# nebarnix/Project-Desert-Tortoise

Measured on AMD Instinct MI355X. Metric: IQ Msamples/s end-to-end (WAV→minorframes), 1-GPU + %HBM roofline, higher is better.
Workload: dtype f32

## Files before the change

project-desert-tortoise_amd/csrc/pdt_api.hip:

```cpp
#include "pdt_rt.h"
#include "pdt_analytic.h"
#include "pdt_ddc.h"
#include "pdt_survey.h"
#include "pdt_bursts.h"

#include <pthread.h>
#include <sched.h>
#include <sys/mman.h>
#include <sys/stat.h>
#include <sys/syscall.h>

namespace pdtrt {
PDT_CHAIN_INSTANCES(extern, float)
PDT_CHAIN_INSTANCES(extern, double)
std::atomic<long long> g_alloc_ns{0};
hipError_t analytic_launch(hipStream_t st, int fmt, const void *x, long long lo, long long hi, unsigned long long n_out, unsigned long long g0,
                           uint32_t step, const float *tab_dev, void *out);
size_t survey_part_floats(uint64_t nseg, int nfft);
hipError_t survey_launch(hipStream_t st, int fmt, const void *x, uint64_t nseg, int nfft, const float *win, const float *tw, float *part, float *out);
int survey_plan(const pdt_survey_cfg *cfg, double mode_range_hz, double channel_rate, uint64_t nframes, int cap, pdt::SurveyPlan *p);
int survey_carriers(const float *P, const pdt::SurveyPlan &p, double in_rate, pdt_carrier *found);
hipError_t waterfall_launch(hipStream_t st, int fmt, const void *x, uint64_t nrows, int rows_per, int nfft, const float *win, const float *tw, float *rows);
hipError_t row_peaks_launch(hipStream_t st, const float *rows, uint64_t nrows, int nfft, float level, int gb, void *peaks, int *counts);
int bursts_plan(const pdt_bursts_cfg *cfg, double mode_range_hz, double channel_rate, double in_rate, uint64_t nframes, int cap, pdt::BurstPlan *p);
pdt::SurveyPlan bursts_survey_plan(const pdt::BurstPlan &p, const pdt_bursts_cfg *cfg, uint64_t nframes);
int bursts_link(const void *peaks, const int *counts, bool compact, const pdt::BurstPlan &p, double floor, double in_rate, pdt_burst *found, int cap);
hipError_t ddc_launch(hipStream_t st, int fmt, const void *x, long long lo, long long hi, unsigned long long n_out, unsigned long long g0,
                      int decim, const float *taps_dev, const float *tab_dev, const uint32_t *steps, void *const *outs, int k);
}

static std::atomic<int> g_open_contexts{0};
static std::mutex g_link_mu[64];

static std::mutex g_dev_mu;
static std::map<std::string, std::string> g_dev;
void Tuning::load()
{
    std::lock_guard<std::mutex> lock(g_dev_mu);
    if (g_dev.empty()) return;
    auto get = [&](const char *n) -> const char * { auto it = g_dev.find(n); return it == g_dev.end() ? nullptr : it->second.c_str(); };
    if (const char *e = get("PDT_PLL_WARM_SCALE")) pll_warm_scale = atof(e);
    if (const char *e = get("PDT_HEAD_TAUS")) head_taus = atof(e);
    if (const char *e = get("PDT_BAND_PAD")) band_pad = atof(e);
    if (const char *e = get("PDT_PLL_WARM_S")) pll_warm_s = atof(e);
    if (const char *e = get("PDT_AGC_WARM_S")) agc_warm_s = atof(e);
    if (const char *e = get("PDT_AGC_K")) agc_k = atof(e);
    if (const char *e = get("PDT_AGC_TPB")) agc_tpb = std::max(1, atoi(e));
    if (const char *e = get("PDT_PLL_BLOCK")) pll_block = atoi(e);
    if (const char *e = get("PDT_HBM_LIMIT_MB")) hbm_limit_mb = std::max(1ll, atoll(e));
    if (const char *e = get("PDT_BURST_SLAB_ROWS")) burst_slab_rows = std::max(1ll, atoll(e));
    if (const char *e = get("PDT_WINDOW_PIECE")) window_piece = std::max(1ll, atoll(e));
    if (const char *e = get("PDT_SCOUT_SYMS")) scout_syms = std::max(16, atoi(e));
    if (const char *e = get("PDT_FIR_WG_PER_CU")) fir_wg_per_cu = std::min(4096, std::max(1, atoi(e)));
    if (const char *e = get("PDT_INGEST_THREADS")) ingest_threads = std::min(128, std::max(1, atoi(e)));
    if (const char *e = get("PDT_INGEST_SPAN_MB")) ingest_span_mb = std::min(256, std::max(1, atoi(e)));
    if (const char *e = get("PDT_INGEST_STREAMS")) ingest_streams = std::min(4, std::max(1, atoi(e)));
    if (const char *e = get("PDT_INGEST_DIRECT")) ingest_direct = atoi(e) ? 1 : 0;
    if (const char *e = get("PDT_INGEST_NUMA")) ingest_numa = atoi(e) ? 1 : 0;
    if (const char *e = get("PDT_FIX_PASSES")) fix_passes = atoi(e);
    if (const char *e = get("PDT_GSEG")) gseg = std::min(64, std::max(2, atoi(e)));
    if (const char *e = get("PDT_GSPAN")) gspan = std::min(256, std::max(1, atoi(e)));
    if (const char *e = get("PDT_GSPAN_CAP")) gspan_cap = std::max(64, atoi(e));
    fir_generic = get("PDT_FIR_GENERIC") != nullptr;
    mix_unfused = get("PDT_MIX_UNFUSED") != nullptr;
    quality_inline = get("PDT_QUALITY_INLINE") != nullptr;
    gardner_nostride = get("PDT_GARDNER_NOSTRIDE") != nullptr;
    gemit_groups = get("PDT_GEMIT_GROUPS") != nullptr;
    agc_unfused = get("PDT_AGC_UNFUSED") != nullptr;
    manch_3pass = get("PDT_MANCH_3PASS") != nullptr;
    sync_serial = get("PDT_SYNC_SERIAL") != nullptr;
    agc_lanes = get("PDT_AGC_LANES") != nullptr;
    no_excl = get("PDT_NO_EXCL") != nullptr;
    gardner_onebuf = get("PDT_GARDNER_ONEBUF") != nullptr;
    gardner_noring = get("PDT_GARDNER_NORING") != nullptr;
    ema_noguess = get("PDT_EMA_NOGUESS") != nullptr;
    gardner_sequential = get("PDT_GARDNER_SEQUENTIAL") != nullptr;
    seg_sequential = get("PDT_SEG_SEQUENTIAL") != nullptr;
    overlap = get("PDT_NO_OVERLAP") == nullptr;
    if (const char *e = get("PDT_OVERLAP_SPLIT")) {
        int k = 0;
        for (const char *q = e; *q && k < 8; k++) {
            char *end = nullptr;
            overlap_split[k] = strtod(q, &end);
            if (end == q) break;
            q = (*end == ',') ? end + 1 : end;
        }
    }
    chain_one_range = get("PDT_CHAIN_ONE_RANGE") != nullptr;
    debug_overlap = get("PDT_DEBUG_OVERLAP") != nullptr;
    if (const char *e = get("PDT_OVERLAP_SEGMENTS")) overlap_segments = std::min(64, std::max(1, atoi(e)));
    if (const char *e = get("PDT_OVERLAP_MIN_MB")) overlap_min_mb = std::min(1 << 20, std::max(1, atoi(e)));
    debug_sync = get("PDT_DEBUG_SYNC") != nullptr;
    pll_noshort = get("PDT_PLL_NOSHORT") != nullptr;
    pll_nockpt = get("PDT_PLL_NOCKPT") != nullptr;
    pll_noconsensus = get("PDT_PLL_NOCONSENSUS") != nullptr;
    pll_notail = get("PDT_PLL_NOTAIL") != nullptr;
    seg_plain = get("PDT_SEG_PLAIN") != nullptr;
    sync_block = get("PDT_SYNC_BLOCK") != nullptr;
}

namespace pdtrt {

int execute_plans(pdt_ctx *const *ctxs, int M)
{
    pdt_ctx *L0 = ctxs[0];
    HIP_TRY(hipSetDevice(L0->cfg.device));
    const Plan &P0 = L0->plan;
    for (int m = 1; m < M; m++)
        if (!P0.same_shape(ctxs[m]->plan)) return PDT_ERR_STATE;
    const size_t per = P0.packs.size();
    const size_t total = per * (size_t)M;
    int rc;
    if ((rc = L0->packs_dev.ensure(total + 64))) return rc;
    if (total + 64 > L0->packs_pin_cap) {
        if (L0->packs_pin) (void)hipHostFree(L0->packs_pin);
        L0->packs_pin = nullptr;
        L0->packs_pin_cap = 0;
        const size_t want = 2 * total + 4096;
        if (timed_host_malloc((void **)&L0->packs_pin, want) != hipSuccess) { (void)hipGetLastError(); return PDT_ERR_NOMEM; }
        L0->packs_pin_cap = want;
    }
    unsigned char *pin = (unsigned char *)L0->packs_pin;
    for (const PlanOp &o : P0.ops) {
        if (o.op != OP_LAUNCH) continue;
        for (int m = 0; m < M; m++)
            memcpy(pin + (size_t)M * o.pack_off + (size_t)m * o.pack_size, ctxs[m]->plan.packs.data() + o.pack_off, o.pack_size);
    }
    hipStream_t st[2] = { L0->stream, L0->stream2 };
    if (total) HIP_TRY(hipMemcpyAsync(L0->packs_dev.p, pin, total, hipMemcpyHostToDevice, st[0]));
    Launcher T(L0);
    const unsigned char *dev = (const unsigned char *)L0->packs_dev.p;
    for (size_t i = 0; i < P0.ops.size(); i++) {
        const PlanOp &o = P0.ops[i];
        switch (o.op) {
        case OP_LAUNCH: {
            dim3 g = o.grid;
            for (int m = 1; m < M; m++) {
                const dim3 gm = ctxs[m]->plan.ops[i].grid;
                g.x = std::max(g.x, gm.x);
                g.y = std::max(g.y, gm.y);
            }
            g.z = (unsigned)M;
            o.go(g, o.block, o.shmem, st[o.side], dev + (size_t)M * o.pack_off);
            if (L0->tune.debug_sync) {
                const hipError_t e = hipStreamSynchronize(st[o.side]);
                fprintf(stderr, "libpdt: [%zu] %s grid (%u,%u,%u) block %u lds %zu: %s\n", i, o.name, g.x, g.y, g.z, o.block.x, o.shmem,
                        hipGetErrorString(e));
            }
            break;
        }
        case OP_MEMSET:
            for (int m = 0; m < M; m++) {
                const PlanOp &om = ctxs[m]->plan.ops[i];
                if (om.bytes) HIP_TRY(hipMemsetAsync(om.dst, om.value, om.bytes, st[om.side]));
            }
            T.gap();
            break;
        case OP_D2H:
        case OP_H2D:
            for (int m = 0; m < M; m++) {
                const PlanOp &om = ctxs[m]->plan.ops[i];
                if (om.bytes)
                    HIP_TRY(hipMemcpyAsync(om.dst, om.src, om.bytes, o.op == OP_D2H ? hipMemcpyDeviceToHost : hipMemcpyHostToDevice, st[0]));
            }
            T.gap();
            break;
        case OP_FORK:
            HIP_TRY(hipEventRecord(L0->ev_fork, st[0]));
            HIP_TRY(hipStreamWaitEvent(st[1], L0->ev_fork, 0));
            break;
        case OP_JOIN_RECORD: HIP_TRY(hipEventRecord(L0->ev_join, st[1])); break;
// ... 2294 lines not shown
```

project-desert-tortoise_amd/csrc/pdt_chain.inc:

```
#include "pdt_rt.h"

namespace pdtrt {
PDT_WIDE_INSTANCES(extern, float)
PDT_WIDE_INSTANCES(extern, double)

template <typename T> int finish_capture(pdt_ctx *ctx, uint64_t n, const FinishArgs &FA)
{
    const bool argos = FA.argos, need_lock = FA.need_lock, fuse_mix = FA.fuse_mix;
    const long long N = FA.N, n_out = FA.n_out, chunk = FA.chunk, chunk_out = FA.chunk_out, first = FA.first, first_out = FA.first_out,
                    sym_cap = FA.sym_cap;
    const int interp = FA.interp, ntaps = FA.ntaps;
    const uint32_t hit_cap = FA.hit_cap, frame_cap = FA.frame_cap;
    const SyncParams &SP = FA.SP;
    const T Fs = (T)ctx->cfg.sample_rate;
    StreamCarry *seg = ctx->sc.active ? &ctx->sc : nullptr;
    FrameRec *d_frames = (FrameRec *)ctx->frames.p;
    (void)first_out;
    if (!ctx->pending || ctx->pend_n != n) return PDT_ERR_STATE;
    ctx->pending = false;
    pdt_ctx *lead = ctx->leader ? ctx->leader : ctx;
    if (seg && seg->in_place && !ctx->tune.sync_block) {
        for (;;) {
            const hipError_t e = hipEventQuery(lead->ev1);
            if (e == hipSuccess) break;
// ... 1112 lines not shown
        if constexpr (std::is_same<T, float>::value) {
            std::vector<unsigned> cand;
            std::vector<int> mfirst((size_t)GD.n_q + 1);
            cand.reserve((size_t)GD.n_q * 2);
            for (int m = 0; m < GD.n_q; m++) {
                mfirst[(size_t)m] = (int)cand.size();
                const float q = GD.q_min + (float)m * GD.u;
                const float fr = q - floorf(q);
                if (fr <= 0.61f) cand.push_back((unsigned)(2 * m));
                if (fr >= 0.39f) cand.push_back((unsigned)(2 * m + 1));
            }
            mfirst[(size_t)GD.n_q] = (int)cand.size();
            GD.n_cand = (int)cand.size();
            const long long key = chunk_out * 1000003ll + (long long)llround((double)GP.step * 4096.0);
            if ((rc = ctx->gcand.ensure(cand.size() * sizeof(unsigned)))) return rc;
            if ((rc = ctx->gmfirst.ensure(mfirst.size() * sizeof(int)))) return rc;
            if (ctx->gcand_key != key) {
                HIP_TRY(hipMemcpyAsync(ctx->gcand.p, cand.data(), cand.size() * sizeof(unsigned), hipMemcpyHostToDevice, st));
                HIP_TRY(hipMemcpyAsync(ctx->gmfirst.p, mfirst.data(), mfirst.size() * sizeof(int), hipMemcpyHostToDevice, st));
                HIP_TRY(hipStreamSynchronize(st));
                ctx->gcand_key = key;
            }
            const long long n_tab = (n_chunks - 1) / GD.span;
            const long long n_groups = n_tab + 1;
            SamplerCarry<float> tab_carry;
            tab_carry.a = (float)carry_in.a; tab_carry.b = (float)carry_in.b; tab_carry.c = (float)carry_in.c;
            tab_carry.c_first = carry_in.c_first; tab_carry.count0 = carry_in.count0;
            SamplerCarry<float> chain_carry = tab_carry;
            chain_carry.c_first = tab_carry.c_first / GD.span;
            const long long g_first = chain_carry.c_first;
            if ((rc = ctx->gtable.ensure((size_t)n_tab * (size_t)(2 * GD.n_q) * sizeof(unsigned)))) return rc;
            if ((rc = ctx->gentries.ensure((size_t)n_chunks * sizeof(GardnerEntry<float>)))) return rc;
            if ((rc = ctx->gbands.ensure((size_t)n_tab * sizeof(GardnerBand)))) return rc;
            L.begin("gardner_table");
            if ((rc = ctx->gclist.ensure((size_t)n_tab * PDT_GTAB_LIST * sizeof(unsigned)))) return rc;
            const int scout_syms = ctx->tune.scout_syms > 0 ? ctx->tune.scout_syms : 455;
            const int scout_tail = (int)std::min<long long>(PDT_GTAB_TAIL, std::max<long long>(256, (long long)((double)scout_syms * (double)GP.step) + 16));
            PDT_LAUNCH(64, k_gardner_scout, dim3((unsigned)n_tab), dim3(64), 0, st, (const float *)d_agc, GP, GD, n_tab,
                               (const int *)ctx->gmfirst.p, (const unsigned *)ctx->gcand.p, (unsigned *)ctx->gtable.p,
                               (GardnerBand *)ctx->gbands.p, (unsigned *)ctx->gclist.p, d_sc->gstats, scout_tail);
            {
                {
                    const unsigned parts = (unsigned)((GD.n_cand + PDT_GTM_SLOTS - 1) / PDT_GTM_SLOTS);
                    PDT_LAUNCH(PDT_GTM_THREADS, (k_gardner_table_merge<PDT_GTAB_WIN>), dim3((unsigned)n_tab, parts), dim3(PDT_GTM_THREADS), 0, st,
                                       (const float *)d_agc, GP, GD, n_tab, (const unsigned *)ctx->gcand.p,
                                       (const GardnerBand *)ctx->gbands.p, (const unsigned *)ctx->gclist.p,
                                       (unsigned *)ctx->gtable.p, d_sc->gstats);
                }
                if (GD.span > 1) {
                    const unsigned cap_keys = ctx->tune.gspan_cap ? (unsigned)ctx->tune.gspan_cap
                                                                  : (unsigned)std::min<long long>(std::max<long long>(n_tab * 128, 1ll << 20), 1ll << 28);
                    const size_t cap_items = (size_t)cap_keys / PDT_GSUB_KEYS + (size_t)n_tab + 1;
                    if ((rc = ctx->gspan_keys.ensure((size_t)cap_keys * sizeof(unsigned)))) return rc;
                    if ((rc = ctx->gspan_tails.ensure((size_t)cap_keys * sizeof(unsigned)))) return rc;
                    if ((rc = ctx->gspan_recs.ensure((size_t)cap_keys * (size_t)(GD.span - 1) * sizeof(GardnerSpanRec)))) return rc;
                    if ((rc = ctx->gspan_rows.ensure((size_t)n_tab * sizeof(GardnerSpanRow)))) return rc;
                    if ((rc = ctx->gspan_items.ensure(cap_items * sizeof(GardnerSpanItem)))) return rc;
                    if ((rc = ctx->gspan_ctl.ensure(sizeof(GardnerSpanCtl)))) return rc;
                    PL.memset_async(ctx->gspan_ctl.p, 0, sizeof(GardnerSpanCtl));
                    PDT_LAUNCH(256, k_gardner_span_keys, dim3((unsigned)n_tab), dim3(256), 0, st, GD, n_tab, (const unsigned *)ctx->gcand.p,
                                       (GardnerBand *)ctx->gbands.p, (const unsigned *)ctx->gclist.p, (const unsigned *)ctx->gtable.p,
                                       (unsigned *)ctx->gspan_keys.p, cap_keys, (GardnerSpanRow *)ctx->gspan_rows.p,
                                       (GardnerSpanItem *)ctx->gspan_items.p, (GardnerSpanCtl *)ctx->gspan_ctl.p);
                    const unsigned walkers = (unsigned)std::min<long long>(n_tab / PDT_GSUB + 64, 256ll * 16);
                    PDT_LAUNCH(64, (k_gardner_span_walk<PDT_GSUB_WIN>), dim3(walkers), dim3(64), 0, st, (const float *)d_agc, GP, GD,
                                       (const unsigned *)ctx->gspan_keys.p, (const GardnerSpanItem *)ctx->gspan_items.p,
                                       (GardnerSpanCtl *)ctx->gspan_ctl.p, (unsigned *)ctx->gspan_tails.p, (GardnerSpanRec *)ctx->gspan_recs.p);
                    PDT_LAUNCH(128, k_gardner_span_join, dim3((unsigned)n_tab), dim3(128), 0, st, GD, n_tab, (const unsigned *)ctx->gcand.p,
                                       (const GardnerBand *)ctx->gbands.p, (const unsigned *)ctx->gclist.p, (unsigned *)ctx->gtable.p,
                                       (const unsigned *)ctx->gspan_keys.p, (const unsigned *)ctx->gspan_tails.p,
                                       (const GardnerSpanRow *)ctx->gspan_rows.p, d_sc->gstats);
                }
            }
            L.end();
            int G = (n_groups < 8000) ? 32 : 64;
            if (ctx->tune.gseg) G = ctx->tune.gseg;
            const long long n_seg = (n_groups + G - 1) / G;
            if ((rc = ctx->gsegmap.ensure((size_t)n_seg * (size_t)(2 * GD.n_q) * sizeof(GardnerSegCell)))) return rc;
            if ((rc = ctx->gsegstart.ensure((size_t)n_seg * sizeof(GardnerSegStart)))) return rc;
            L.begin("gardner_chain");
            PL.memset_async(ctx->gsegstart.p, 0, (size_t)n_seg * sizeof(GardnerSegStart));
            PDT_LAUNCH(1024, k_gardner_segmap, dim3((unsigned)n_seg), dim3(1024), 0, st, (const unsigned *)ctx->gtable.p, GD, n_groups,
                               G, (GardnerSegCell *)ctx->gsegmap.p, (const GardnerBand *)ctx->gbands.p);
            const int n_ranges = (!seg && n_groups >= 8192 && GD.span == 1 && !ctx->tune.chain_one_range) ? 4 : 1;
            if ((rc = ctx->gchain.ensure(sizeof(GardnerChainState)))) return rc;
            const bool side = n_ranges > 1;
            hipStream_t st_emit = side ? ctx->stream2 : st;
            L.end();
            long long c_lo = 0;
            for (int r = 0; r < n_ranges; r++) {
                const long long c_hi = (r == n_ranges - 1) ? n_groups : (n_groups * (r + 1) / n_ranges) / G * G;
                L.begin("gardner_chain");
                PDT_LAUNCH(256, k_gardner_chain, dim3(1), dim3(256), 0, st,
                                   (const float *)d_agc, GP, GD, n_groups,
                                   (const unsigned *)ctx->gtable.p, (const GardnerSegCell *)ctx->gsegmap.p, G,
                                   (GardnerSegStart *)ctx->gsegstart.p, (GardnerEntry<float> *)ctx->gentries.p, d_sc->gstats,
                                   (const GardnerBand *)ctx->gbands.p, n_tab, chain_carry, (seg && seg->have_sampler) ? 1 : 0, c_hi,
                                   (GardnerChainState *)ctx->gchain.p, r == 0 ? 1 : 0,
                                   (const unsigned *)(GD.span > 1 ? ctx->gspan_keys.p : nullptr), (const unsigned *)(GD.span > 1 ? ctx->gspan_tails.p : nullptr),
                                   (const GardnerSpanRow *)(GD.span > 1 ? ctx->gspan_rows.p : nullptr));
                L.end();
                if (side) PL.simple(OP_FORK);
                const long long s_lo = c_lo / G, s_hi = (c_hi + G - 1) / G;
                L.begin("gardner", st_emit);
                if (s_hi > s_lo)
                    PDT_LAUNCH(64, k_gardner_segfill, dim3((unsigned)(s_hi - s_lo)), dim3(64), 0, st_emit, (const float *)d_agc, GP, GD, n_groups,
                                       (const unsigned *)ctx->gtable.p, G, (const GardnerSegStart *)ctx->gsegstart.p,
                                       (GardnerEntry<float> *)ctx->gentries.p, s_lo);
                const unsigned char *d_flags = nullptr;
                if (GD.span > 1 && 8 * (long long)GP.step + 256 < PDT_GEMIT_SUB_WIN && !ctx->tune.gemit_groups &&
                    (double)PDT_GEMIT_SUB_WIN / ((double)GP.step - 0.2) + 2.0 < (double)PDT_GSUB_OUT) {
                    if ((rc = ctx->gcentries.ensure((size_t)n_chunks * sizeof(GardnerEntry<float>)))) return rc;
                    if ((rc = ctx->gflags.ensure((size_t)n_groups + 64))) return rc;
                    PL.memset_async(ctx->gflags.p, 1, (size_t)n_groups, PL.side_of(st_emit));
                    PDT_LAUNCH(64, (k_gardner_emit_first<PDT_GEMIT_SUB_WIN>), dim3((unsigned)((n_tab - g_first + 3) / 4)), dim3(64), 0, st_emit, (const float *)d_agc, GP, GD,
                                       n_tab, (const GardnerEntry<float> *)ctx->gentries.p, (const unsigned *)ctx->gspan_keys.p,
                                       (const GardnerSpanRow *)ctx->gspan_rows.p, (const GardnerSpanRec *)ctx->gspan_recs.p,
                                       (GardnerEntry<float> *)ctx->gcentries.p, (unsigned char *)ctx->gflags.p, (float *)d_sym, d_symidx, sym_cap, g_first);
                    PDT_LAUNCH(64, (k_gardner_emit_rest<PDT_GEMIT_SUB_WIN>), dim3((unsigned)(((n_tab - g_first) * (GD.span - 1) + 3) / 4)), dim3(64), 0, st_emit,
                                       (const float *)d_agc, GP, GD, n_tab, (const GardnerEntry<float> *)ctx->gcentries.p,
                                       (const unsigned char *)ctx->gflags.p, (float *)d_sym, d_symidx, sym_cap, g_first);
                    d_flags = (const unsigned char *)ctx->gflags.p;
                }
                if (c_hi > c_lo)
                    PDT_LAUNCH(256, (k_gardner<float, PDT_GEMIT_LEN, PDT_GEMIT_OUT>), dim3((unsigned)(c_hi - c_lo)), dim3(PDT_GARDNER_THREADS), 0, st_emit,
                                       (const float *)d_agc, (const float *)d_lock, GP, (float *)d_sym, d_symidx, &d_sc->nsym, sym_cap,
                                       (const GardnerEntry<float> *)ctx->gentries.p, tab_carry, (SamplerCarry<float> *)d_carry_out, c_lo, GD.span, d_flags);
                L.end();
                c_lo = c_hi;
            }
            if (side) {
                PL.simple(OP_JOIN_RECORD);
                PL.simple(OP_JOIN_WAIT);
            }
        }
        return PDT_OK;
    }

    int rec_sampler()
    {
        int rc = PDT_OK;
        (void)rc;
        if (use_table) {
            if ((rc = rec_sampler_table())) return rc;
        } else if (use_mm) {
            MmParams<T> MP;
            const T rangeT = (T)(ctx->cfg.mm_step_range != 0 ? ctx->cfg.mm_step_range : 3.0);
            MP.kp = (T)(ctx->cfg.mm_kp != 0 ? ctx->cfg.mm_kp : 0.15);
            MP.step0 = (T)(int)fsi / baud;
            MP.step_max = (T)(int)fsi / (baud - rangeT);
            MP.step_min = (T)(int)fsi / (baud + rangeT);
            MP.n_total = n_out;
            MP.chunk_out = chunk_out;
            L.begin("gardner");
            if (seg && !seg->have_sampler) carry_in.b = MP.step0;
            PDT_LAUNCH(PDT_GARDNER_THREADS, (k_mm<T, 8192, 1024>), dim3(1), dim3(PDT_GARDNER_THREADS), 0, st, (const T *)d_agc, MP, d_sym, d_symidx,
                               &d_sc->nsym, sym_cap, carry_in, seg ? 1 : 0, d_carry_out);
            L.end();
        } else {
            L.begin("gardner");
            constexpr int SMALL_LEN = 32768 / (int)sizeof(T), SMALL_OUT = 1024;
            const long long small_need = chunk_out + 2 * (long long)GP.step + 24;
            const double small_syms = (double)chunk_out / ((double)GP.step - 0.25) + 4.0;
            constexpr int RING_LEN = 20480 / (int)sizeof(T), RING_NB = 6, RING_OUT = 256;
            if (small_need <= RING_LEN && small_syms < RING_OUT && chunk_out >= 4 * (long long)GP.step + 8 && n_chunks >= 8 && !seg &&
                !ctx->tune.gardner_onebuf && !ctx->tune.gardner_noring) {
                const size_t need_bytes = ((size_t)n_chunks + 64 + 15) & ~(size_t)15;
                if ((rc = ctx->gneed.ensure(need_bytes + (size_t)n_chunks * sizeof(CalmEntry<T>)))) return rc;
                CalmEntry<T> *d_calm = (CalmEntry<T> *)((char *)ctx->gneed.p + need_bytes);
                PDT_LAUNCH(256, k_chunk_need<T>, dim3((unsigned)n_chunks), dim3(256), 0, st, (const T *)d_agc, n_out, chunk_out, n_chunks,
                                   (unsigned char *)ctx->gneed.p);
                T gran_scale = 0;
                if (!ctx->tune.gardner_nostride) {
                    const double top = (double)chunk_out + 2.0 * (double)GP.step + 2.0;
                    const int E = ilogb(top) + 1, p = sizeof(T) == 8 ? 53 : 24;
                    const T sc = (T)ldexp(1.0, p - E);
                    const T gstep = GP.step * sc;
                    if (E < p && gstep == (T)rint((double)gstep) && (double)gstep < ldexp(1.0, p - 1)) gran_scale = sc;
                }
                PDT_LAUNCH(64 * (RING_NB + 1), (k_gardner_ring<T, RING_LEN, RING_NB, RING_OUT>), dim3(1), dim3(64 * (RING_NB + 1)), 0, st,
                                   (const T *)d_agc, (const T *)d_lock, GP, (const unsigned char *)ctx->gneed.p, d_sym, d_symidx, &d_sc->nsym,
                                   sym_cap, d_calm, gran_scale);
                PDT_LAUNCH(256, k_calm_emit<T>, dim3((unsigned)((n_chunks + 255) / 256)), dim3(256), 0, st, (const unsigned char *)ctx->gneed.p,
                                   (const CalmEntry<T> *)d_calm, GP, d_sym, d_symidx, sym_cap);
            } else if (small_need <= SMALL_LEN && small_syms < SMALL_OUT && !ctx->tune.gardner_onebuf && !seg)
                PDT_LAUNCH(256, (k_gardner_small<T, SMALL_LEN, SMALL_OUT>), dim3(1), dim3(256), 0, st, (const T *)d_agc, (const T *)d_lock, GP,
                                   d_sym, d_symidx, &d_sc->nsym, sym_cap);
            else
                PDT_LAUNCH(256, (k_gardner<T, GardnerLds<T>::LEN, GardnerLds<T>::OUT>), dim3(1), dim3(256), 0, st, d_agc, d_lock, GP, d_sym, d_symidx,
                                   &d_sc->nsym, sym_cap, (const GardnerEntry<T> *)nullptr, carry_in, d_carry_out, 0ll, 1, (const unsigned char *)nullptr);
            L.end();
        }

        return PDT_OK;
    }

    int rec_bits()
    {
        int rc = PDT_OK;
        (void)rc;
        L.begin("manchester");
        if (ctx->tune.manch_3pass) {
            PDT_LAUNCH(PDT_TILE_THREADS, k_manch_tile<T>, dim3((unsigned)n_tiles), dim3(PDT_TILE_THREADS), 0, st, d_sym, &d_sc->nsym, manch_thr,
                               d_tiles, sym_pad);
// ... 580 lines not shown
```

project-desert-tortoise_amd/csrc/pdt_kernels_back.h:

```cpp
#pragma once
#include "pdt_device_math.h"

namespace pdt {

template <typename T> struct alignas(16) Vec16 {
    static constexpr int N = 16 / sizeof(T);
    T v[N];
};

template <typename T> struct GardnerParams {
    T step, kp, lim;
    long long n_total;
    long long chunk_out;
    int argos_heap;
    unsigned long long argos_field_bits;
    int argos_even;
};

template <typename T>
__device__ __forceinline__ T gardner_beyond(const T *__restrict__ in, const T *__restrict__ lock, const GardnerParams<T> &P,
                                            long long c, long long n_cur, long long idx)
{
    const long long C = P.chunk_out;
    if (idx < C)
// ... 1431 lines not shown
            emit(cur, (unsigned)rn);
            const float err = __builtin_amdgcn_fmed3f(kp * (cur - L.prev) * mid, -lim, lim);
            L.ns = L.ns - err;
            L.q_last = L.ns;
            L.half = L.ns + hs;
            L.ns = L.ns + step;
            L.prev = cur;
            L.i_last = (unsigned)rn;
            L.count++;
        }
        flush();
        if (last_window) break;
        enter_hi = stop + step + 1.2f;
        wbase = wend - margin - back;
    }
}


template <int WIN>
__device__ __forceinline__ void k_gardner_span_walk(const float *__restrict__ in, GardnerParams<float> P, GardnerDomain D,
                                                    const unsigned *__restrict__ keys, const GardnerSpanItem *__restrict__ items,
                                                    GardnerSpanCtl *__restrict__ ctl, unsigned *__restrict__ tails,
                                                    GardnerSpanRec *__restrict__ recs )
{
    __shared__ __attribute__((aligned(16))) float win[PDT_GSUB * WIN];
    __shared__ float s_ref[3];
    __shared__ unsigned s_next;
    const int lane = threadIdx.x;
    const int mysub = lane / PDT_GSUB_KEYS, sublane = lane % PDT_GSUB_KEYS;
    const float nT = (float)P.chunk_out;
    const unsigned n_items = ctl->items;
    for (;;) {
        __syncthreads();
        if (lane == 0) s_next = atomicAdd(&ctl->cursor, (unsigned)PDT_GSUB);
        __syncthreads();
        const unsigned q0 = s_next;
        if (q0 >= n_items) break;
        long long c_sub[PDT_GSUB];
        GardnerSpanItem mine = items[q0];
#pragma unroll
        for (int u = 0; u < PDT_GSUB; u++) {
            const GardnerSpanItem it = (q0 + (unsigned)u < n_items) ? items[q0 + u] : items[q0];
            c_sub[u] = (long long)it.row * D.span + 1;
            if (mysub == u) {
                mine = it;
                if (q0 + (unsigned)u >= n_items) mine.cnt = 0;
            }
        }
        GardnerLane L;
        L.q_last = 0; L.i_last = 0; L.count = 0; L.k = 0;
        L.active = (unsigned)sublane < mine.cnt;
        L.ns = L.prev = L.half = 0;
        long long my_c = 0;
#pragma unroll
        for (int u = 0; u < PDT_GSUB; u++) my_c = (mysub == u) ? c_sub[u] : my_c;
        if (L.active) gardner_entry_from_candidate(in, P, D, my_c, (int)keys[mine.first + sublane], L.ns, L.prev, L.half);
        if (lane == 0) { s_ref[0] = L.ns; s_ref[1] = L.prev; s_ref[2] = L.half; }
        __syncthreads();
        if (!L.active) { L.ns = s_ref[0]; L.prev = s_ref[1]; L.half = s_ref[2]; }
        for (int g = 1; g < D.span; g++) {
            long long cc[PDT_GSUB];
#pragma unroll
            for (int u = 0; u < PDT_GSUB; u++) cc[u] = c_sub[u] + (g - 1);
            if (L.active) {
                GardnerSpanRec rc;
                rc.ns = L.ns; rc.prev = L.prev; rc.half = L.half; rc.count = L.count;
                recs[(size_t)(mine.first + sublane) * (size_t)(D.span - 1) + (size_t)(g - 1)] = rc;
            }
            gardner_sub_chunk<WIN, PDT_GSUB, false>(win, in, P, cc, L, nullptr, nullptr, 0, 0);
            if (g + 1 < D.span) L.ns = L.ns - nT;
        }
        if (L.active) tails[mine.first + sublane] = gardner_encode_exit(D, L.q_last, L.i_last, L.count);
    }
}

#define PDT_GEMIT_SUB_WIN 512
template <int WIN>
__device__ __forceinline__ void k_gardner_emit_first(const float *__restrict__ in, GardnerParams<float> P, GardnerDomain D,
                                                     long long n_rows, const GardnerEntry<float> *__restrict__ entries,
                                                     const unsigned *__restrict__ keys, const GardnerSpanRow *__restrict__ rows,
                                                     const GardnerSpanRec *__restrict__ recs,
                                                     GardnerEntry<float> *__restrict__ centries, unsigned char *__restrict__ flags,
                                                     float *__restrict__ sym, long long *__restrict__ symidx, long long sym_cap,
                                                     long long g_first = 0 )
{
    __shared__ __attribute__((aligned(16))) float win[4 * WIN];
    const int lane = threadIdx.x;
    const int mysub = lane >> 4;
    const long long g0 = g_first + (long long)blockIdx.x * 4;
    if (g0 >= n_rows) return;
    long long c_sub[4];
#pragma unroll
    for (int u = 0; u < 4; u++) c_sub[u] = ((g0 + u < n_rows) ? g0 + u : g0) * D.span;
    const long long my_g = (g0 + mysub < n_rows) ? g0 + mysub : g0;
    const GardnerEntry<float> e = entries[my_g];
    GardnerLane L;
    L.ns = e.ns; L.prev = e.prev; L.half = e.half; L.q_last = 0; L.i_last = 0; L.count = 0; L.k = 0;
    L.active = g0 + mysub < n_rows;
    __shared__ float o_val[4 * PDT_GSUB_OUT];
    __shared__ unsigned o_idx[4 * PDT_GSUB_OUT];
    gardner_sub_chunk<WIN, 4, true>(win, in, P, c_sub, L, sym, symidx, e.offset, sym_cap, o_val, o_idx);
    if (L.active && (lane & 15) == 0) {
        unsigned char flag = 1;
        const GardnerSpanRow rw = rows[my_g];
        const unsigned cell = gardner_encode_exit(D, L.q_last, L.i_last, L.count);
        if (rw.n != ~0u && rw.n > 0 && cell != PDT_GTAB_MISS) {
            const unsigned k1 = cell & ((1u << D.idx_bits) - 1u);
            unsigned lo = 0, hi = rw.n;
            while (lo < hi) {
                const unsigned mid = (lo + hi) >> 1;
                if (keys[rw.off + mid] < k1) lo = mid + 1;
                else hi = mid;
            }
            if (lo < rw.n && keys[rw.off + lo] == k1) {
                const GardnerSpanRec *rc = recs + (size_t)(rw.off + lo) * (size_t)(D.span - 1);
                for (int q = 1; q < D.span; q++) {
                    GardnerEntry<float> ce;
                    ce.ns = rc[q - 1].ns; ce.prev = rc[q - 1].prev; ce.half = rc[q - 1].half;
                    ce.offset = e.offset + (long long)L.count + (long long)rc[q - 1].count;
                    centries[my_g * D.span + q] = ce;
                }
                flag = 0;
            }
        }
        flags[my_g] = flag;
    }
}

template <int WIN>
__device__ __forceinline__ void k_gardner_emit_rest(const float *__restrict__ in, GardnerParams<float> P, GardnerDomain D,
                                                    long long n_rows, const GardnerEntry<float> *__restrict__ centries,
                                                    const unsigned char *__restrict__ flags, float *__restrict__ sym,
                                                    long long *__restrict__ symidx, long long sym_cap, long long g_first = 0)
{
    __shared__ __attribute__((aligned(16))) float win[4 * WIN];
    const int lane = threadIdx.x;
    const int mysub = lane >> 4;
    const long long per = D.span - 1;
    const long long total = n_rows * per;
    const long long i0 = g_first * per + (long long)blockIdx.x * 4;
    if (i0 >= total) return;
    long long c_sub[4];
    bool live[4];
    long long c_any = -1;
#pragma unroll
    for (int u = 0; u < 4; u++) {
        const long long i = i0 + u;
        const long long g = (i < total) ? i / per : 0;
        live[u] = i < total && !flags[g];
        c_sub[u] = g * D.span + 1 + (i - g * per);
        if (live[u] && c_any < 0) c_any = c_sub[u];
    }
    if (c_any < 0) return;
#pragma unroll
    for (int u = 0; u < 4; u++) c_sub[u] = live[u] ? c_sub[u] : c_any;
    long long my_c = c_any;
    bool mine_live = false;
#pragma unroll
    for (int u = 0; u < 4; u++)
        if (mysub == u) { my_c = c_sub[u]; mine_live = live[u]; }
    const GardnerEntry<float> e = centries[my_c];
    GardnerLane L;
    L.ns = e.ns; L.prev = e.prev; L.half = e.half; L.q_last = 0; L.i_last = 0; L.count = 0; L.k = 0;
    L.active = mine_live;
    __shared__ float o_val[4 * PDT_GSUB_OUT];
    __shared__ unsigned o_idx[4 * PDT_GSUB_OUT];
    gardner_sub_chunk<WIN, 4, true>(win, in, P, c_sub, L, sym, symidx, e.offset, sym_cap, o_val, o_idx);
}

__device__ __forceinline__ void k_gardner_span_join(GardnerDomain D, long long n_rows, const unsigned *__restrict__ cand_k,
                                                    const GardnerBand *__restrict__ bands, const unsigned *__restrict__ clist,
                                                    unsigned *__restrict__ table, const unsigned *__restrict__ keys,
                                                    const unsigned *__restrict__ tails, const GardnerSpanRow *__restrict__ rows,
                                                    unsigned *__restrict__ stats )
{
    const long long r = blockIdx.x;
    if (r >= n_rows) return;
    const GardnerSpanRow rw = rows[r];
    if (rw.n == ~0u) return;
    const long long c0 = r * D.span;
    const GardnerBand bd = bands[r];
    const unsigned *cand = bd.listed ? (clist + (size_t)r * PDT_GTAB_LIST) : cand_k;
    unsigned *row = table + (size_t)r * (size_t)(2 * D.n_q);
    const unsigned kmask = (1u << D.idx_bits) - 1u;
    for (int j = bd.j_lo + (int)threadIdx.x; j < bd.j_hi; j += (int)blockDim.x) {
        const unsigned k = (c0 == 0) ? 0u : cand[j];
        const unsigned cell = row[k];
        if (cell == PDT_GTAB_MISS) continue;
        const unsigned k1 = cell & kmask;
        unsigned lo = 0, hi = rw.n;
        while (lo < hi) {
            const unsigned mid = (lo + hi) >> 1;
            if (keys[rw.off + mid] < k1) lo = mid + 1;
            else hi = mid;
        }
        unsigned out = PDT_GTAB_MISS;
        if (lo < rw.n && keys[rw.off + lo] == k1) {
            const unsigned tail = tails[rw.off + lo];
            if (tail != PDT_GTAB_MISS) {
                const unsigned cnt = (cell >> D.idx_bits) + (tail >> D.idx_bits);
                if (cnt < (1u << (32 - D.idx_bits)) - 1u) out = (tail & kmask) | (cnt << D.idx_bits);
            }
        }
        if (out == PDT_GTAB_MISS) atomicAdd(&stats[0], 1u);
        row[k] = out;
    }
}

__device__ __forceinline__ unsigned gardner_cell(const unsigned *__restrict__ table, size_t stride, const GardnerBand &b,
                                                 long long c, unsigned key)
{
    const unsigned cell = table[(size_t)c * stride + key];
    return (key >= b.k_lo && key <= b.k_hi) ? cell : PDT_GTAB_MISS;
}

struct GardnerSegCell { unsigned next, count; };
struct GardnerSegStart { unsigned key; unsigned hopped; long long offset; };

__device__ __forceinline__ void k_gardner_segmap(const unsigned *__restrict__ table, GardnerDomain D, long long n_groups,
                                                          int G, GardnerSegCell *__restrict__ segmap,
// ... 1315 lines not shown
```

project-desert-tortoise_amd/csrc/pdt_rt.h:

```cpp
#ifndef PDT_RT_H
#define PDT_RT_H
#include <hip/hip_runtime.h>
#include <math.h>
#include <stdio.h>
#include <stdlib.h>
#include <string.h>

#include <errno.h>
#include <fcntl.h>
#include <unistd.h>

#include <algorithm>
#include <functional>
#include <map>
#include <mutex>
#include <atomic>
#include <chrono>
#include <memory>
#include <new>
#include <string>
#include <thread>
#include <type_traits>
#include <vector>

// ... 143 lines not shown

typedef void (*GoFn)(dim3, dim3, size_t, hipStream_t, const void *);
enum { OP_LAUNCH, OP_MEMSET, OP_FORK, OP_JOIN_RECORD, OP_JOIN_WAIT, OP_TBEGIN, OP_TEND, OP_TGAP, OP_D2H, OP_H2D, OP_EV0, OP_EV1 };
struct PlanOp {
    int op = OP_LAUNCH, side = 0;
    GoFn go = nullptr;
    dim3 grid, block;
    size_t shmem = 0, pack_off = 0, pack_size = 0;
    void *dst = nullptr;
    const void *src = nullptr;
    int value = 0;
    size_t bytes = 0;
    const char *name = nullptr;
};
struct Plan {
    std::vector<PlanOp> ops;
    std::vector<unsigned char> packs;
    hipStream_t side_stream = nullptr;
    void clear() { ops.clear(); packs.clear(); }
    int side_of(hipStream_t s) const { return (side_stream && s == side_stream) ? 1 : 0; }
    template <auto Body, int TB, typename... A> void launch(const char *kname, dim3 grid, dim3 block, size_t shmem, int side, A &&...args)
    {
        using PackT = typename BodyTraits<decltype(Body)>::pack;
        static_assert(std::is_trivially_copyable<PackT>::value, "kernel arguments travel as plain bytes");
        PackT pk;
        memset((void *)&pk, 0, sizeof pk);
        pack_fill(pk, args...);
        PlanOp o;
        o.op = OP_LAUNCH;
        o.name = kname;
        o.side = side;
        o.grid = grid;
        o.block = block;
        o.shmem = shmem;
        o.pack_off = (packs.size() + 15) & ~(size_t)15;
        o.pack_size = sizeof(PackT);
        static_assert(alignof(PackT) <= 16, "pack alignment");
        packs.resize(o.pack_off + o.pack_size, 0);
        memcpy(packs.data() + o.pack_off, &pk, sizeof pk);
        o.go = &go_fn<Body, TB>;
        ops.push_back(o);
    }
    void simple(int op, int side = 0, const char *name = nullptr)
    {
        PlanOp o;
        o.op = op; o.side = side; o.name = name;
        ops.push_back(o);
    }
    void memset_async(void *dst, int value, size_t bytes, int side = 0)
    {
        PlanOp o;
        o.op = OP_MEMSET; o.side = side; o.dst = dst; o.value = value; o.bytes = bytes;
        ops.push_back(o);
    }
    void copy(int op, void *dst, const void *src, size_t bytes)
    {
        PlanOp o;
        o.op = op; o.dst = dst; o.src = src; o.bytes = bytes;
        ops.push_back(o);
    }
    bool same_shape(const Plan &o) const
    {
        if (ops.size() != o.ops.size() || packs.size() != o.packs.size()) return false;
        for (size_t i = 0; i < ops.size(); i++) {
            const PlanOp &a = ops[i], &b = o.ops[i];
            if (a.op != b.op || a.side != b.side || a.go != b.go || a.block.x != b.block.x || a.block.y != b.block.y ||
                a.shmem != b.shmem || a.pack_off != b.pack_off || a.pack_size != b.pack_size)
                return false;
        }
        return true;
    }
};
#define PDT_LAUNCH(TB, KERNEL, grid, block, shmem, stream, ...) \
    PL.launch<&KERNEL, TB>(#KERNEL, grid, block, shmem, PL.side_of(stream), __VA_ARGS__)

}
using namespace pdtrt;

struct Tuning {
    double band_pad = 0.0, pll_warm_scale = 1.0, head_taus = 0.0, agc_k = 0.0, pll_warm_s = 0.0, agc_warm_s = 0.0;
    double overlap_split[8] = { 0, 0, 0, 0, 0, 0, 0, 0 };
    long long hbm_limit_mb = 0, window_piece = 0, burst_slab_rows = 0;
    int ingest_direct = -1, ingest_numa = -1;
    int scout_syms = 0, gspan = 0, gspan_cap = 0, ingest_threads = 0, ingest_span_mb = 0, ingest_streams = 0, overlap_segments = 0, overlap_min_mb = 0, fir_wg_per_cu = 0, agc_tpb = 0, gseg = 0, pll_block = 0, fix_passes = 2;
    bool fir_generic = false, mix_unfused = false, quality_inline = false, gemit_groups = false, agc_unfused = false, no_excl = false, gardner_onebuf = false, gardner_noring = false, gardner_sequential = false, seg_sequential = false, agc_lanes = false, overlap = true, debug_overlap = false, chain_one_range = false, ema_noguess = false, debug_sync = false, pll_noshort = false, pll_nockpt = false, pll_noconsensus = false, pll_notail = false, seg_plain = false, sync_block = false, gardner_nostride = false, manch_3pass = false, sync_serial = false;
    void load();
};

struct StreamCarry {
    bool active = false;
    bool final_seg = false;
    bool in_place = false;
    uint64_t place_align = 0;
    bool quality = false;
    long long first = 0;
    uint64_t origin = 0;
    bool have_norm = false;
    double norm_factor = 0, gain = 0;
    bool locked = false;
    double phase = 0, freq = 0, avg = 0, locksig = 0, sweep = 0;
    int64_t lock_sample = -1;
    double lock_freq_hz = 0, avg_at_lock = 0;
    bool have_sampler = false;
    double sa = 0, sb = 0, sc = 0;
    double sym_m2 = 0, sym_m1 = 0;
    unsigned clockmod = 0;
    uint64_t nsym_total = 0;
    std::vector<unsigned char> kept_bits;
    std::vector<long long> kept_src;
    uint64_t bit_base = 0;
    uint64_t nbits_total = 0;
    long long next_free = 0;
    bool have_pending = false;
    pdt_frame pending;
    std::vector<pdt_frame> seg_frames;
    uint64_t seg_new_symbols = 0, seg_new_bits = 0;
};

enum { IN_NONE = 0, IN_IQ, IN_REAL, IN_WB };
struct InFmt {
    int kind;
    int code;
    int bytes;
    int pcm_fmt;
    int pcm_bytes;
};
inline InFmt in_fmt(int sample_format)
{
    switch (sample_format) {
    case PDT_FMT_PCM16: return { IN_IQ, sample_format, 4, 0, 4 };
    case PDT_FMT_F32: return { IN_IQ, sample_format, 8, 1, 8 };
    case PDT_FMT_REAL_PCM16: return { IN_REAL, sample_format, 2, 1, 8 };
    case PDT_FMT_REAL_F32: return { IN_REAL, sample_format, 4, 1, 8 };
    case PDT_FMT_WB_PCM16: return { IN_WB, sample_format, 4, 1, 8 };
    case PDT_FMT_WB_F32: return { IN_WB, sample_format, 8, 1, 8 };
    case PDT_FMT_WB_CU8:
    case PDT_FMT_WB_CS8: return { IN_WB, sample_format, 2, 1, 8 };
    }
    return { IN_NONE, sample_format, 0, 0, 0 };
}

struct HaloCarry {
    DevBuf buf[2];
    int cur = 0;
    uint64_t left = 0, pending = 0, in = 0, out = 0;
};

struct pdt_ctx {
    pdt_config cfg;
    pdt_loop_params lp = {};
    Tuning tune;
    StreamCarry sc;
    int elem;
    uint32_t interp, ntaps;
    hipStream_t stream = nullptr;
    bool own_stream = false;
    hipEvent_t ev0 = nullptr, ev1 = nullptr, ev_fork = nullptr, ev_join = nullptr;
    hipStream_t stream2 = nullptr;

    DevBuf pcm, pll, lock, fir, agc, sym, symidx, bits, bitsym, hits, frames, taps, mag, seams_pll, seams_agc, scal, lockinfo, term, seams_ema, gtable, gentries, gcand, gmfirst, stiles, gsegmap, gsegstart, gbands, gclist, gneed, gchain, gspan_keys, gspan_tails, gspan_rows, gspan_items, gspan_ctl, gspan_recs, gcentries, gflags, agc_maps, pll_head, taps_rot, pll_scratch, tip, sync_scr, agc_raw, agc_ckpt, pll_ckpt;
    bool counted = false;
    bool keep_agc_raw = false;
    bool keep_quality = false;
    bool keep_pll_asked = false;
    bool keep_pll = true;
    DevBuf avgph, term_ap, seams_q, chunkinfo;
    struct PllInject {
// ... 295 lines not shown
```

Baseline: 52120.

## Split Gardner chain into ranges for span>1 and overlap per-range emit

Turns on multi-range splitting of the sequential Gardner chain kernel when span>1 (threshold 4096 groups), and adds a tunable range count. The emit_first/emit_rest kernels now process only the group slice of each range on the side stream, so symbol emission can run alongside the chain for later ranges. The flags memset and buffer setup move out of the loop. The cost is extra launches, cross-stream ordering, and a risk that the range boundaries interact wrongly with the per-group flags.

```diff
diff --git a/project-desert-tortoise_amd/csrc/pdt_api.hip b/project-desert-tortoise_amd/csrc/pdt_api.hip
--- a/project-desert-tortoise_amd/csrc/pdt_api.hip
+++ b/project-desert-tortoise_amd/csrc/pdt_api.hip
@@ -87,6 +87,7 @@
         }
     }
     chain_one_range = get("PDT_CHAIN_ONE_RANGE") != nullptr;
+    if (const char *e = get("PDT_CHAIN_RANGES")) chain_ranges = std::min(64, std::max(1, atoi(e)));
     debug_overlap = get("PDT_DEBUG_OVERLAP") != nullptr;
     if (const char *e = get("PDT_OVERLAP_SEGMENTS")) overlap_segments = std::min(64, std::max(1, atoi(e)));
     if (const char *e = get("PDT_OVERLAP_MIN_MB")) overlap_min_mb = std::min(1 << 20, std::max(1, atoi(e)));
diff --git a/project-desert-tortoise_amd/csrc/pdt_chain.inc b/project-desert-tortoise_amd/csrc/pdt_chain.inc
--- a/project-desert-tortoise_amd/csrc/pdt_chain.inc
+++ b/project-desert-tortoise_amd/csrc/pdt_chain.inc
@@ -1218,11 +1218,20 @@
             PL.memset_async(ctx->gsegstart.p, 0, (size_t)n_seg * sizeof(GardnerSegStart));
             PDT_LAUNCH(1024, k_gardner_segmap, dim3((unsigned)n_seg), dim3(1024), 0, st, (const unsigned *)ctx->gtable.p, GD, n_groups,
                                G, (GardnerSegCell *)ctx->gsegmap.p, (const GardnerBand *)ctx->gbands.p);
-            const int n_ranges = (!seg && n_groups >= 8192 && GD.span == 1 && !ctx->tune.chain_one_range) ? 4 : 1;
+            int n_ranges = (!seg && n_groups >= (GD.span == 1 ? 8192 : 4096)) ? 4 : 1;
+            if (!seg && ctx->tune.chain_ranges > 0) n_ranges = (int)std::min<long long>(ctx->tune.chain_ranges, std::max<long long>(1, n_groups / G));
+            if (ctx->tune.chain_one_range) n_ranges = 1;
             if ((rc = ctx->gchain.ensure(sizeof(GardnerChainState)))) return rc;
             const bool side = n_ranges > 1;
             hipStream_t st_emit = side ? ctx->stream2 : st;
             L.end();
+            const bool emit_chunks = GD.span > 1 && 8 * (long long)GP.step + 256 < PDT_GEMIT_SUB_WIN && !ctx->tune.gemit_groups &&
+                                     (double)PDT_GEMIT_SUB_WIN / ((double)GP.step - 0.2) + 2.0 < (double)PDT_GSUB_OUT;
+            if (emit_chunks) {
+                if ((rc = ctx->gcentries.ensure((size_t)n_chunks * sizeof(GardnerEntry<float>)))) return rc;
+                if ((rc = ctx->gflags.ensure((size_t)n_groups + 64))) return rc;
+                PL.memset_async(ctx->gflags.p, 1, (size_t)n_groups, PL.side_of(st_emit));
+            }
             long long c_lo = 0;
             for (int r = 0; r < n_ranges; r++) {
                 const long long c_hi = (r == n_ranges - 1) ? n_groups : (n_groups * (r + 1) / n_ranges) / G * G;
@@ -1244,18 +1253,17 @@
                                        (const unsigned *)ctx->gtable.p, G, (const GardnerSegStart *)ctx->gsegstart.p,
                                        (GardnerEntry<float> *)ctx->gentries.p, s_lo);
                 const unsigned char *d_flags = nullptr;
-                if (GD.span > 1 && 8 * (long long)GP.step + 256 < PDT_GEMIT_SUB_WIN && !ctx->tune.gemit_groups &&
-                    (double)PDT_GEMIT_SUB_WIN / ((double)GP.step - 0.2) + 2.0 < (double)PDT_GSUB_OUT) {
-                    if ((rc = ctx->gcentries.ensure((size_t)n_chunks * sizeof(GardnerEntry<float>)))) return rc;
-                    if ((rc = ctx->gflags.ensure((size_t)n_groups + 64))) return rc;
-                    PL.memset_async(ctx->gflags.p, 1, (size_t)n_groups, PL.side_of(st_emit));
-                    PDT_LAUNCH(64, (k_gardner_emit_first<PDT_GEMIT_SUB_WIN>), dim3((unsigned)((n_tab - g_first + 3) / 4)), dim3(64), 0, st_emit, (const float *)d_agc, GP, GD,
-                                       n_tab, (const GardnerEntry<float> *)ctx->gentries.p, (const unsigned *)ctx->gspan_keys.p,
-                                       (const GardnerSpanRow *)ctx->gspan_rows.p, (const GardnerSpanRec *)ctx->gspan_recs.p,
-                                       (GardnerEntry<float> *)ctx->gcentries.p, (unsigned char *)ctx->gflags.p, (float *)d_sym, d_symidx, sym_cap, g_first);
-                    PDT_LAUNCH(64, (k_gardner_emit_rest<PDT_GEMIT_SUB_WIN>), dim3((unsigned)(((n_tab - g_first) * (GD.span - 1) + 3) / 4)), dim3(64), 0, st_emit,
-                                       (const float *)d_agc, GP, GD, n_tab, (const GardnerEntry<float> *)ctx->gcentries.p,
-                                       (const unsigned char *)ctx->gflags.p, (float *)d_sym, d_symidx, sym_cap, g_first);
+                if (emit_chunks) {
+                    const long long g_lo = std::max(g_first, c_lo), g_hi = std::min(c_hi, n_tab);
+                    if (g_hi > g_lo) {
+                        PDT_LAUNCH(64, (k_gardner_emit_first<PDT_GEMIT_SUB_WIN>), dim3((unsigned)((g_hi - g_lo + 3) / 4)), dim3(64), 0, st_emit, (const float *)d_agc, GP, GD,
+                                           n_tab, (const GardnerEntry<float> *)ctx->gentries.p, (const unsigned *)ctx->gspan_keys.p,
+                                           (const GardnerSpanRow *)ctx->gspan_rows.p, (const GardnerSpanRec *)ctx->gspan_recs.p,
+                                           (GardnerEntry<float> *)ctx->gcentries.p, (unsigned char *)ctx->gflags.p, (float *)d_sym, d_symidx, sym_cap, g_lo, g_hi);
+                        PDT_LAUNCH(64, (k_gardner_emit_rest<PDT_GEMIT_SUB_WIN>), dim3((unsigned)(((g_hi - g_lo) * (GD.span - 1) + 3) / 4)), dim3(64), 0, st_emit,
+                                           (const float *)d_agc, GP, GD, n_tab, (const GardnerEntry<float> *)ctx->gcentries.p,
+                                           (const unsigned char *)ctx->gflags.p, (float *)d_sym, d_symidx, sym_cap, g_lo, g_hi);
+                    }
                     d_flags = (const unsigned char *)ctx->gflags.p;
                 }
                 if (c_hi > c_lo)
diff --git a/project-desert-tortoise_amd/csrc/pdt_kernels_back.h b/project-desert-tortoise_amd/csrc/pdt_kernels_back.h
--- a/project-desert-tortoise_amd/csrc/pdt_kernels_back.h
+++ b/project-desert-tortoise_amd/csrc/pdt_kernels_back.h
@@ -1537,11 +1537,13 @@
                                                      const GardnerSpanRec *__restrict__ recs,
                                                      GardnerEntry<float> *__restrict__ centries, unsigned char *__restrict__ flags,
                                                      float *__restrict__ sym, long long *__restrict__ symidx, long long sym_cap,
-                                                     long long g_first = 0 )
+                                                     long long g_first ,
+                                                     long long g_end )
 {
     __shared__ __attribute__((aligned(16))) float win[4 * WIN];
     const int lane = threadIdx.x;
     const int mysub = lane >> 4;
+    if (g_end < n_rows) n_rows = g_end;
     const long long g0 = g_first + (long long)blockIdx.x * 4;
     if (g0 >= n_rows) return;
     long long c_sub[4];
@@ -1586,11 +1588,13 @@
 __device__ __forceinline__ void k_gardner_emit_rest(const float *__restrict__ in, GardnerParams<float> P, GardnerDomain D,
                                                     long long n_rows, const GardnerEntry<float> *__restrict__ centries,
                                                     const unsigned char *__restrict__ flags, float *__restrict__ sym,
-                                                    long long *__restrict__ symidx, long long sym_cap, long long g_first = 0)
+                                                    long long *__restrict__ symidx, long long sym_cap, long long g_first,
+                                                    long long g_end )
 {
     __shared__ __attribute__((aligned(16))) float win[4 * WIN];
     const int lane = threadIdx.x;
     const int mysub = lane >> 4;
+    if (g_end < n_rows) n_rows = g_end;
     const long long per = D.span - 1;
     const long long total = n_rows * per;
     const long long i0 = g_first * per + (long long)blockIdx.x * 4;
diff --git a/project-desert-tortoise_amd/csrc/pdt_rt.h b/project-desert-tortoise_amd/csrc/pdt_rt.h
--- a/project-desert-tortoise_amd/csrc/pdt_rt.h
+++ b/project-desert-tortoise_amd/csrc/pdt_rt.h
@@ -249,7 +249,7 @@
     double overlap_split[8] = { 0, 0, 0, 0, 0, 0, 0, 0 };
     long long hbm_limit_mb = 0, window_piece = 0, burst_slab_rows = 0;
     int ingest_direct = -1, ingest_numa = -1;
-    int scout_syms = 0, gspan = 0, gspan_cap = 0, ingest_threads = 0, ingest_span_mb = 0, ingest_streams = 0, overlap_segments = 0, overlap_min_mb = 0, fir_wg_per_cu = 0, agc_tpb = 0, gseg = 0, pll_block = 0, fix_passes = 2;
+    int scout_syms = 0, gspan = 0, gspan_cap = 0, ingest_threads = 0, ingest_span_mb = 0, ingest_streams = 0, overlap_segments = 0, overlap_min_mb = 0, fir_wg_per_cu = 0, agc_tpb = 0, gseg = 0, pll_block = 0, fix_passes = 2, chain_ranges = 0;
     bool fir_generic = false, mix_unfused = false, quality_inline = false, gemit_groups = false, agc_unfused = false, no_excl = false, gardner_onebuf = false, gardner_noring = false, gardner_sequential = false, seg_sequential = false, agc_lanes = false, overlap = true, debug_overlap = false, chain_one_range = false, ema_noguess = false, debug_sync = false, pll_noshort = false, pll_nockpt = false, pll_noconsensus = false, pll_notail = false, seg_plain = false, sync_block = false, gardner_nostride = false, manch_3pass = false, sync_serial = false;
     void load();
 };
```

After: 50440. 3.2% lower.
